# cloudflare/flow-pipeline

Hardware: AMD Instinct MI355X
Metric: FlowMessages/sec aggregated into flows_5m (higher is better)
Workload: dtype u64

## Files before the change

flow-pipeline_amd/csrc/flowagg.hip:

```cpp
#include <hip/hip_runtime.h>
#include <sched.h>
#include <hipcub/hipcub.hpp>

#include <algorithm>
#include <atomic>
#include <thread>
#include <chrono>
#include <cmath>
#include <condition_variable>
#include <functional>
#include <map>
#include <cstdio>
#include <cstdlib>
#include <cstring>
#include <ctime>
#include <memory>
#include <mutex>
#include <string>
#include <vector>

#include "../../include/flowagg.h"
#include "bucket_range.h"
#include "buffers.h"
#include "kernels.cuh"
// ... 66 lines not shown
        uint32_t* tail() const { return counts + wcounts_cap(counts); }
        uint32_t nwg = 0, wcapq = 0, wplog2 = 0, wmask = 0, wm = 0;
        size_t wregion = 0;
        uint64_t n = 0;
        uint32_t minb = 0, maxb = 0;
        bool minb_known = false;
    };
    std::vector<WChunk> wlog, wlog_free;
    bool wide_probed = false;
    bool wide_defer = false;
    uint64_t seen_wfold = 0;
    size_t wlog_max = 8;
    uint64_t wpot_total = 0, known_wpot = 0;
    uint64_t snap_wpot[NSNAP] = {};
    uint32_t wseg_budget = 0;
    uint32_t late_below = 0;
    uint64_t wlog_recorded = 0, wlog_folded = 0, wlog_replayed = 0, wlog_dropped = 0, wlog_wm_moves = 0, wlog_nomem_folds = 0;
    bool wide_scatter = true;
    uint64_t seen_wused = 0, seen_ok_w = 0;
    bool cms_atomic = false;
    bool cms_scatter_ok = false;
    int sink_mode = 0;
    int t8_mode = 0;
    uint64_t t8_wide_until = 0;
    uint64_t seen_misfit8 = 0, seen_ok = 0;
    uint64_t seen_retried = 0, seq_until = 0;
    int seq_mode = 0;
    uint64_t seen_agg_groups = 0, seen_agg_launches = 0;
    uint32_t agg_passes_forced = 0;
    uint32_t agg_passes = 1;
    unsigned stage_threads = 8;
    uint32_t par = 0;
    uint32_t seg_cap_limit = 0;
    uint32_t last_nwg = 0;
    uint32_t plog2 = PART_LOG2_MAX, wgpc_cap = 0;

    PinnedBuf<uint8_t> h_stage[2];
    hipEvent_t stage_ev[2] = {nullptr, nullptr};
    int stage_cur = 0;
    DevBuf<uint8_t> d_in[2];

    DevBuf<> col_block;
    ColumnPtrs cols{};

    DevBuf<> rc_buf;
    DevBuf<> rw_buf;
    DevBuf<> m_scratch;
    DevBuf<> m_out[2];
    DevBuf<> cut_buf;
    hipStream_t copy_stream = nullptr;
    hipStream_t cand_stream = nullptr;
    hipEvent_t cand_ev[2] = {nullptr, nullptr};
    DevBuf<> fs_scratch;
    DevBuf<> fs_off;
    DevBuf<> wl_scratch;
    DevBuf<> part_buf;
    DevBuf<unsigned int> part_cnt;
    DevBuf<> xch_buf;
    uint32_t group_members = 0;
    PinnedBuf<> h_rows;
    hipEvent_t copy_ev[2] = {nullptr, nullptr};

    DevBuf<unsigned long long> cms_src, cms_dst;
    size_t cms_words = 0;
    bool cms_dirty = false;
    DevBuf<unsigned long long> cms_src_m, cms_dst_m;
// ... 77 lines not shown
    a.tab = c->tab;
    a.mask = (1u << c->cap_log2) - 1;
    a.rlog2 = as_rlog2(c->cap_log2);
    a.spill = c->spill;
    a.spill_cap = c->spill_cap;
    a.ctr = c->d_ctr;
    a.exotic_idx = c->d_exotic;
    a.cms_src = c->cms_src;
    a.cms_dst = c->cms_dst;
    a.cms_depth = c->cfg.cms_depth;
    a.cms_wl2 = c->cfg.cms_width_log2;
    a.cms_seed = c->cfg.cms_seed;
    a.ks_src = c->ks_src;
    a.ks_dst = c->ks_dst;
    a.ks_mask = (1u << c->ks_log2) - 1;
    a.cand_src = c->cand_bits[0];
    a.cand_dst = c->cand_bits[1];
    a.cms_nrep = c->cand_state ? 1u : CMS_REPLICAS;
    a.cols = c->cols;
    a.dbg = c->dbg;
    a.tile_recs = BLOCK;
    a.retry_idx = c->d_exotic ? c->d_exotic + c->exotic_cap() : nullptr;
    a.key_sets = c->cfg.key_sets;
    a.wtab = c->wtab;
    a.wmask = (1u << c->wcap_log2) - 1;
    a.wplog2 = wide_plog2(c->wcap_log2);
    a.wspill = c->wspill;
    a.wspill_cap = c->wspill_cap;
    a.port_hist = c->port_hist;
    a.gran_recip = (1.0 / (double)c->gran) * (1.0 + 1.0 / 1099511627776.0);
    a.par = c->par;
    a.agg_passes = c->agg_passes_forced ? c->agg_passes_forced : c->agg_passes;
    a.late_below = c->late_below;
    return a;
}

template <class K>
static int grid_for(fa_ctx* c, K kernel, uint32_t n, uint32_t tile_recs) {
    uint32_t tiles = (n + tile_recs - 1) / tile_recs;
    int per_cu = 0;
    if (hipOccupancyMaxActiveBlocksPerMultiprocessor(&per_cu, kernel, BLOCK, 0) != hipSuccess || per_cu < 1)
        per_cu = 2;
    if (c->wgpc_cap && (int)c->wgpc_cap < per_cu) per_cu = (int)c->wgpc_cap;
    uint32_t g = std::min<uint32_t>((uint32_t)c->num_cus * (uint32_t)per_cu, SEG_MAX_NWG);
    return (int)std::max(1u, std::min(tiles, g));
}

extern "C" int fa_create(const fa_config* cfg_in, fa_ctx** out) {
    if (!cfg_in || !out) {
        g_create_error = "fa_create: null argument";
        return FA_ERR_ARG;
    }
    *out = nullptr;
    int ndev = 0;
    if (hipGetDeviceCount(&ndev) != hipSuccess || ndev <= 0) {
        g_create_error = "fa_create: no HIP device (libflowagg has no CPU fallback)";
        return FA_ERR_NO_DEVICE;
    }
    fa_config cfg = *cfg_in;
    if (cfg.window_secs == 0) cfg.window_secs = 300;
    if (cfg.table_capacity_log2 == 0) cfg.table_capacity_log2 = 20;
    if (cfg.cms_depth == 0) cfg.cms_depth = 4;
    if (cfg.cms_width_log2 == 0) cfg.cms_width_log2 = 20;
    if (cfg.key_sets == 0) cfg.key_sets = FA_KEYS_AS_PAIR;
    if (cfg.topk_capacity_log2 == 0) cfg.topk_capacity_log2 = 20;
    if (cfg.wide_capacity_log2 == 0) cfg.wide_capacity_log2 = 20;
    if (cfg.topk_track == 0) cfg.topk_track = 256;
    if (cfg.max_batch_records == 0) cfg.max_batch_records = AGG_MAX_BATCH;
    if (cfg.max_batch_records > AGG8_MAX_BATCH) cfg.max_batch_records = AGG8_MAX_BATCH;
    uint32_t gran = cfg.subwindow_secs ? cfg.subwindow_secs : cfg.window_secs;
    if (cfg.device < 0 || cfg.device >= ndev || gran < 60 || 86400 % gran != 0 ||
        cfg.window_secs % gran != 0 || 86400 % cfg.window_secs != 0 || cfg.table_capacity_log2 < 10 ||
        cfg.table_capacity_log2 > 30 || cfg.cms_depth > 16 || cfg.cms_width_log2 < 4 ||
        cfg.cms_width_log2 > 28 || (cfg.key_sets & ~63u) || cfg.topk_mode > FA_TOPK_CANDIDATES || cfg.topk_capacity_log2 < 8 || cfg.topk_capacity_log2 > 30 ||
        cfg.wide_capacity_log2 < 8 || cfg.wide_capacity_log2 > 30) {
        g_create_error = "fa_create: invalid configuration";
        return FA_ERR_ARG;
    }
    fa_ctx* c = new fa_ctx();
    c->cfg = cfg;
    c->gran = gran;
    c->cap_log2 = cfg.table_capacity_log2;
    if (const char* d = getenv("FA_DEBUG_FLAGS")) c->dbg = (uint32_t)strtoul(d, nullptr, 0);
    if (const char* d = getenv("FA_PLOG2")) c->plog2 = std::min<uint32_t>(PART_LOG2_MAX, std::max<uint32_t>(4, (uint32_t)atoi(d)));
    if (const char* d = getenv("FA_WGPC")) c->wgpc_cap = (uint32_t)atoi(d);
    if (const char* d = getenv("FA_SEG_CAP")) c->seg_cap_limit = std::max<uint32_t>(40u, (uint32_t)atoi(d) & ~7u);
    if (const char* d = getenv("FA_SINK")) c->sink_mode = !strcmp(d, "direct") ? 1 : !strcmp(d, "scatter") ? 2 : 0;
    if (const char* d = getenv("FA_CMS")) c->cms_atomic = !strcmp(d, "atomic");
    if (const char* d = getenv("FA_WIDE")) c->wide_mode = !strcmp(d, "atomic") ? 1 : !strcmp(d, "scatter") ? 2 : !strcmp(d, "log") ? 3 : 0;
    if (const char* d = getenv("FA_WIDE_LOG_CHUNKS")) c->wlog_max = (size_t)std::max(0, atoi(d));
    if (const char* d = getenv("FA_WSEG_BUDGET")) c->wseg_budget = (uint32_t)std::max(1, atoi(d));
    if (const char* d = getenv("FA_AGG_PASSES")) {
        const int v = atoi(d);
        c->agg_passes_forced = (v == 1 || v == 2 || v == 4 || v == 8) ? (uint32_t)v : 0u;
    }
    c->cms_scatter_ok = cms_scatterable(cfg.cms_depth, cfg.cms_width_log2);
    if (const char* d = getenv("FA_STAGE_THREADS")) c->stage_threads = (unsigned)std::min(64, std::max(1, atoi(d)));
    c->stage_threads = std::min(c->stage_threads, std::max(1u, std::thread::hardware_concurrency()));
    if (const char* d = getenv("FA_TUPLE")) c->t8_mode = !strcmp(d, "8") ? 1 : !strcmp(d, "16") ? 2 : 0;
    if (const char* d = getenv("FA_SEQ")) c->seq_mode = !strcmp(d, "1") ? 1 : !strcmp(d, "0") ? 2 : 0;
    auto bail = [&](const char* what, hipError_t e) {
        g_create_error = std::string("fa_create: ") + what + ": " + hipGetErrorString(e);
        fa_destroy(c);
        return e == hipErrorOutOfMemory ? FA_ERR_NOMEM : FA_ERR_HIP;
    };
    hipError_t e;
    if ((e = hipSetDevice(cfg.device)) != hipSuccess) return bail("hipSetDevice", e);
    {
        int v = 0;
        if (hipDeviceGetAttribute(&v, hipDeviceAttributeMultiprocessorCount, cfg.device) == hipSuccess && v > 0)
            c->num_cus = v;
    }
    if ((e = hipStreamCreateWithFlags(&c->stream, hipStreamNonBlocking)) != hipSuccess)
        return bail("hipStreamCreate", e);
    for (int i = 0; i < 2; i++)
        if ((e = hipEventCreateWithFlags(&c->stage_ev[i], hipEventDisableTiming)) != hipSuccess ||
            (e = hipEventCreateWithFlags(&c->copy_ev[i], hipEventDisableTiming)) != hipSuccess)
            return bail("hipEventCreate", e);
    for (int i = 0; i < fa_ctx::NSNAP; i++)
        if ((e = hipEventCreateWithFlags(&c->snap_ev[i], hipEventDisableTiming)) != hipSuccess) return bail("hipEventCreate", e);
    if (!c->h_snap.grow(sizeof(Counters) * fa_ctx::NSNAP)) return bail("hipHostMalloc", hipGetLastError());
    c->spill_cap = 2u * cfg.max_batch_records + (1u << 21);
    c->wide_per_record = ((cfg.key_sets & FA_KEYS_ADDR_PORT_PROTO) ? 1u : 0u) + ((cfg.key_sets & FA_KEYS_PORT_HIST) ? 2u : 0u) +
                         ((cfg.key_sets & FA_KEYS_MINUTE_SERIES) ? 1u : 0u);
    c->wspill_cap = (uint32_t)std::min<uint64_t>((uint64_t)c->wide_per_record * 2u * cfg.max_batch_records + (1u << 21), 1u << 25);
    size_t tab_bytes = sizeof(Slot) << c->cap_log2;
    if (!c->tab.grow(tab_bytes)) return bail("hipMalloc(table)", hipGetLastError());
    if ((e = hipMemsetAsync(c->tab, 0, tab_bytes, c->stream)) != hipSuccess) return bail("memset", e);
    if (!c->spill.grow(sizeof(SpillEntry) * c->spill_cap))
        return bail("hipMalloc(spill)", hipGetLastError());
    if (!c->d_ctr.grow(sizeof(Counters))) return bail("hipMalloc(ctr)", hipGetLastError());
    if ((e = hipMemsetAsync(c->d_ctr, 0, sizeof(Counters), c->stream)) != hipSuccess)
        return bail("memset", e);
    if (!c->h_ctr.grow(sizeof(Counters))) return bail("hipHostMalloc", hipGetLastError());
    if (cfg.key_sets & (FA_KEYS_SRCADDR_CMS | FA_KEYS_DSTADDR_CMS)) {
        c->cms_words = (size_t)cfg.cms_depth << cfg.cms_width_log2;
        if (cfg.key_sets & FA_KEYS_SRCADDR_CMS) {
            if (!c->cms_src.grow(c->cms_words * 8 * CMS_REPLICAS)) return bail("hipMalloc(cms)", hipGetLastError());
            if ((e = hipMemsetAsync(c->cms_src, 0, c->cms_words * 8 * CMS_REPLICAS, c->stream)) != hipSuccess)
                return bail("memset", e);
        }
        if (cfg.key_sets & FA_KEYS_DSTADDR_CMS) {
            if (!c->cms_dst.grow(c->cms_words * 8 * CMS_REPLICAS)) return bail("hipMalloc(cms)", hipGetLastError());
            if ((e = hipMemsetAsync(c->cms_dst, 0, c->cms_words * 8 * CMS_REPLICAS, c->stream)) != hipSuccess)
                return bail("memset", e);
        }
        if (cfg.topk_mode == FA_TOPK_CANDIDATES) {
            if ((e = hipStreamCreateWithFlags(&c->cand_stream, hipStreamNonBlocking)) != hipSuccess) return bail("hipStreamCreate(side stream)", e);
            for (int i = 0; i < 2; i++)
                if ((e = hipEventCreateWithFlags(&c->cand_ev[i], hipEventDisableTiming)) != hipSuccess) return bail("hipEventCreate", e);
        }
        c->ks_log2 = cfg.topk_capacity_log2;
        const size_t ks_bytes = sizeof(KeySlot) << c->ks_log2;
        if (cfg.key_sets & FA_KEYS_SRCADDR_CMS) {
            if (!c->ks_src.grow(ks_bytes)) return bail("hipMalloc(key set)", hipGetLastError());
            if ((e = hipMemsetAsync(c->ks_src, 0, ks_bytes, c->stream)) != hipSuccess) return bail("memset", e);
        }
        if (cfg.key_sets & FA_KEYS_DSTADDR_CMS) {
            if (!c->ks_dst.grow(ks_bytes)) return bail("hipMalloc(key set)", hipGetLastError());
            if ((e = hipMemsetAsync(c->ks_dst, 0, ks_bytes, c->stream)) != hipSuccess) return bail("memset", e);
        }
        if (cfg.topk_mode == FA_TOPK_CANDIDATES) {
            c->cand_bits_bytes = std::max<size_t>(c->cms_words / 8, 8) + 8;
            for (int d = 0; d < 2; d++)
                if (cfg.key_sets & (d ? FA_KEYS_DSTADDR_CMS : FA_KEYS_SRCADDR_CMS)) {
                    if (!c->cand_bits[d].grow(c->cand_bits_bytes)) return bail("hipMalloc(candidate bits)", hipGetLastError());
                    if ((e = hipMemsetAsync(c->cand_bits[d], 0, c->cand_bits_bytes, c->stream)) != hipSuccess) return bail("memset", e);
// ... 251 lines not shown
```

flow-pipeline_amd/csrc/ingest.cuh:

```cuda
#pragma once
#include <hip/hip_runtime.h>
#include <stdint.h>

#include "sinks.cuh"

#ifndef FA_FOLD_EVERY
#define FA_FOLD_EVERY 4
#endif
#ifndef FA_LT_KEEP
#define FA_LT_KEEP 8u
#endif
namespace fa {

struct NoHook {
    __device__ __forceinline__ void operator()() const {}
};
struct LaneTally {
    uint32_t ok = 0, direct = 0, second = 0, misfit8 = 0, late = 0;
    uint32_t tick = 0;
};
template <int MODE, uint32_t KEYSETS, uint32_t COLS, bool T8 = false, int CANDM = -1, class Hook = NoHook>
__device__ __forceinline__ void lane_work(const KArgs& a, LdsTable<LDS_SLOTS>& lt, LdsMinutes& lm, uint32_t* part_cnt, const uint32_t* tile,
                                          bool mine, uint32_t pos, uint32_t end, uint32_t rec_idx, uint32_t tb_base,
                                          LaneTally& tally, uint32_t& pmode, uint32_t& lt_seen, uint32_t& lt_hits,
                                          uint4* bins, uint32_t* bin_cnt, uint32_t& fill_out, Hook&& after_parse = Hook(),
                                          CmsLds* cl = nullptr, uint32_t* cms_scratch = nullptr, HotAddrs* hot = nullptr,
                                          uint32_t* wpart_cnt = nullptr, uint32_t* seq = nullptr) {
    constexpr uint32_t TB = bin_cap<T8, bin_line(KEYSETS)>();
    bool sure = false, framed_ok = false;
    Rec r;
    rec_clear(r);
    if (mine) {
        LdsSrc src{tile};
        framed_ok = true;
        if (a.framed && !(FA_DBG(a, DBG_NO_FRAME))) {
            uint32_t pl = 0;
// ... 471 lines not shown
};
template <>
struct HotAddrsOpt<false> {
    __device__ __forceinline__ HotAddrs* get() { return nullptr; }
};

template <uint32_t KEYSETS, bool T8, bool SEQ = false, int CANDM = -1>
__global__ __launch_bounds__(wtile_block<KEYSETS>(), wt_lean(KEYSETS) ? 6 : 4) void wtile_kernel(KArgs a) {
    constexpr uint32_t BL = bin_line(KEYSETS);
    constexpr uint32_t TB = bin_cap<T8, BL>();
    constexpr uint32_t COLS = cols_for_keysets<KEYSETS>();
    constexpr int WBLOCK = wtile_block<KEYSETS>();
    constexpr bool HAS_CMS = (KEYSETS & (FA_KEYS_SRCADDR_CMS | FA_KEYS_DSTADDR_CMS)) != 0;
    constexpr int WAVES = WBLOCK / 64;
    constexpr int WT_STRIDE = wtile_stride<KEYSETS>();
    __shared__ CmsLdsOpt<HAS_CMS> cms_lds;
    __shared__ HotAddrsOpt<HAS_CMS> hot_lds;
    __shared__ uint32_t cms_scratch_all[HAS_CMS ? WAVES * 16 : 1];
    __shared__ __attribute__((aligned(16))) uint32_t tiles[WAVES * WT_STRIDE / 4];
    __shared__ __attribute__((aligned(16))) uint4 bins[NPART_MAX * BL];
    __shared__ uint32_t bin_cnt[NPART_MAX];
    __shared__ uint32_t part_cnt[NPART_MAX];
    __shared__ uint32_t flush_scratch[WAVES * 16];
    constexpr bool HAS_APP = (KEYSETS & FA_KEYS_ADDR_PORT_PROTO) != 0;
    __shared__ uint32_t wpart_cnt[HAS_APP ? (1u << WIDE_PLOG2_MAX) + 2u : 1u];
    __shared__ LdsTable<LDS_SLOTS> lt;
    __shared__ LdsMinutes lm;
    constexpr bool HAS_SEQ = SEQ && KEYSETS == FA_KEYS_AS_PAIR;
    static_assert(!SEQ || KEYSETS == FA_KEYS_AS_PAIR, "the learnt-order variant exists for the flows_5m rollup alone");
    __shared__ uint32_t seq_all[HAS_SEQ ? WAVES * (SEQ_MAX + 2) : 1];

    const uint32_t tid = threadIdx.x, lane = tid & 63;
    const uint32_t wave = __builtin_amdgcn_readfirstlane(tid >> 6);
    if (HAS_SEQ && lane < 2) seq_all[wave * (SEQ_MAX + 2) + lane] = 0;
    if (KEYSETS & FA_KEYS_AS_PAIR) {
        lds_table_clear(lt);
        for (int i = tid; i < NPART_MAX; i += WBLOCK) {
            part_cnt[i] = 0;
            bin_cnt[i] = 0;
        }
    }
    if (KEYSETS & FA_KEYS_MINUTE_SERIES) lds_minutes_clear(lm);
    if (HAS_APP)
        for (int i = tid; i < (1 << WIDE_PLOG2_MAX) + 2; i += WBLOCK) wpart_cnt[i] = i < (1 << WIDE_PLOG2_MAX) ? 0u : 0xffffffffu;
    CmsLds* const cl = (HAS_CMS && (CANDM >= 0 || a.cseg)) ? cms_lds.get() : nullptr;
    HotAddrs* const hot = (HAS_CMS && (KEYSETS != KS_ALL || (a.key_sets & (FA_KEYS_SRCADDR_CMS | FA_KEYS_DSTADDR_CMS)))) ? hot_lds.get() : nullptr;
    if (HAS_CMS && cl)
        for (int i = tid; i < (int)(CMS_SETS * CMS_NPART); i += WBLOCK) {
            cl->bin_cnt[i] = 0;
            cl->part_cnt[i] = 0;
        }
    if (HAS_CMS && hot)
        for (int i = tid; i < (int)(CMS_SETS * HOT_SLOTS); i += WBLOCK) {
            const int set = i / HOT_SLOTS, sl = i % HOT_SLOTS;
            const size_t at = (size_t)blockIdx.x * (CMS_SETS * HOT_SLOTS) + i;
            const uint32_t tg = a.hot_seed_tag ? a.hot_seed_tag[at] : 0u;
            if (tg >= 2u) {
                const HotSeed sd = a.hot_seed[at];
                hot->lo[set][sl] = sd.lo;
                hot->hi[set][sl] = sd.hi;
                hot->w[set][sl] = 0;
            }
            hot->touched[set][sl] = 0;
            *hot->tag(set, sl) = tg >= 2u ? tg : 0u;
        }
    uint32_t* tile = tiles + wave * (WT_STRIDE / 4);

    LaneTally tally;
    uint32_t lt_seen = 0, lt_hits = 0, pmode = 0;
    uint32_t tb_base = 0;
    const uint32_t ntiles = (a.n + a.tile_recs - 1) / a.tile_recs;
    __shared__ uint32_t next_k;
    if (tid == 0) next_k = 2u * WAVES;
    const uint32_t wg_pos = (gridDim.x & 7u) == 0u ? (blockIdx.x & 7u) * (gridDim.x >> 3) + (blockIdx.x >> 3) : blockIdx.x;
    auto tile_after_next = [&]() {
        uint32_t k = 0;
        if (lane == 0) k = lds_add_rtn_u32(&next_k, 1u);
        return (uint32_t)__builtin_amdgcn_readfirstlane((int)k) * gridDim.x + wg_pos;
    };
    struct __attribute__((packed, aligned(4))) OffPair {
        uint32_t lo, hi;
    };
    struct Tile {
        uint32_t r0, nrec;
        uint32_t q0, q1;
    };
    auto tile_load = [&](uint32_t t) {
        Tile d{0, 0, 0, 0};
        if (t < ntiles) {
            d.r0 = t * a.tile_recs;
            d.nrec = min(a.tile_recs, a.n - d.r0);
            if (lane < d.nrec) {
                const OffPair v = *reinterpret_cast<const OffPair*>(a.off + d.r0 + lane);
                d.q0 = v.lo;
                d.q1 = v.hi;
            }
        }
        return d;
    };
    constexpr uint32_t CAP = (uint32_t)WT_STRIDE - 16u;
    auto issue_dma = [&](uint32_t lo, uint32_t hi) {
        const uint32_t cbase = lo & ~15u;
        const uint32_t nbytes = hi > cbase ? min(hi - cbase, CAP) : 0u;
        for (uint32_t o = lane * 16u; o < nbytes; o += 1024u)
            __builtin_amdgcn_global_load_lds((const __attribute__((address_space(1))) void*)(a.buf + cbase + o),
                                             (__attribute__((address_space(3))) void*)(tile + (o - lane * 16u) / 4u), 16, 0, 2);
    };
    Tile cur = tile_load(wave * gridDim.x + wg_pos);
    uint32_t cur_lo = (uint32_t)__builtin_amdgcn_readfirstlane((int)cur.q0);
    uint32_t cur_hi = cur.nrec ? min((uint32_t)__builtin_amdgcn_readlane((int)cur.q1, (int)(cur.nrec - 1u)), a.len) : 0u;
    bool live = lane < cur.nrec;
    __syncthreads();
    issue_dma(cur_lo, cur_hi);
    Tile nxt = tile_load((wave + WAVES) * gridDim.x + wg_pos);
    tb_base = probe_tb_base(a);
    if (blockIdx.x == 0 && tid == 0) a.ctr->tb_base = tb_base;
    uint32_t t2 = 0;
    bool t2_have = false;
    while (cur.nrec != 0) {
        dma_wait_all();
        if (!t2_have) {
            t2 = tile_after_next();
            t2_have = true;
        }
        const uint32_t cbase = cur_lo & ~15u;
        const bool valid = live && cur.q1 >= cur.q0 && cur.q0 >= cur_lo && cur.q1 <= cur_hi;
        const bool staged = valid && cur.q1 - cbase <= CAP;
        bool rest = valid && !staged;
        const bool hopeless = (live && !valid) || (rest && cur.q0 == cur_lo);
        if (FA_ANY(hopeless)) {
            if (hopeless) {
                unsigned int j = atomicAdd(&a.ctr->exotic_count[a.par], 1u);
                a.exotic_idx[j] = cur.r0 + lane;
            }
            rest = rest && !hopeless;
        }
        uint32_t fill = 0xffffffffu;
        lane_work<MODE_INGEST, KEYSETS, COLS, T8, CANDM>(a, lt, lm, part_cnt, tile, staged, cur.q0 - cbase, cur.q1 - cbase, cur.r0 + lane, tb_base, tally,
                                                  pmode, lt_seen, lt_hits, bins, bin_cnt, fill, NoHook(), cl, cms_scratch_all + (HAS_CMS ? wave * 16 : 0), hot,
                                                  (HAS_APP && a.wseg) ? wpart_cnt : nullptr, HAS_SEQ ? seq_all + wave * (SEQ_MAX + 2) : nullptr);
        if ((KEYSETS & FA_KEYS_AS_PAIR) && a.seg) bins_flush<T8, BL>(a, bins, bin_cnt, part_cnt, flush_scratch + wave * 16, fill, tb_base, tally.direct);
        const unsigned long long restm = __builtin_amdgcn_ballot_w64(rest);
        if (restm != 0ull) {
            live = rest;
            cur_lo = (uint32_t)__builtin_amdgcn_readlane((int)cur.q0, (int)__builtin_ctzll(restm));
            issue_dma(cur_lo, cur_hi);
            continue;
        }
        t2_have = false;
        cur = nxt;
        cur_lo = (uint32_t)__builtin_amdgcn_readfirstlane((int)cur.q0);
        cur_hi = cur.nrec ? min((uint32_t)__builtin_amdgcn_readlane((int)cur.q1, (int)(cur.nrec - 1u)), a.len) : 0u;
        live = lane < cur.nrec;
        issue_dma(cur_lo, cur_hi);
        nxt = tile_load(t2);
// ... 97 lines not shown
        __syncthreads();
        for (int i = tid; i < (1 << a.wplog2); i += WBLOCK) a.wseg_counts[(size_t)i * a.nwg + blockIdx.x] = min(wpart_cnt[i], a.wcapq);
        if (tid == 0 && wpart_cnt[1u << WIDE_PLOG2_MAX] != 0xffffffffu) {
            atomicMin(&a.ctr->wtb_min, wpart_cnt[1u << WIDE_PLOG2_MAX]);
            atomicMin(&a.ctr->wtb_nmax, wpart_cnt[(1u << WIDE_PLOG2_MAX) + 1u]);
        }
    }
    if (KEYSETS & FA_KEYS_AS_PAIR) {
        __syncthreads();
        for (int i0 = 0; i0 < LDS_SLOTS; i0 += WBLOCK) {
            const int i = i0 + tid;
            Slot* sp = nullptr;
            unsigned long long b = 0, p = 0, c = 0;
            if (i < LDS_SLOTS) {
                const unsigned long long k0 = lt.k0[i], k1 = lt.k1[i];
                b = lt.bytes[i];
                p = lt.packets[i];
                c = lt.count[i];
                if (k0 != 0 && k1 != 0 && c != 0) {
                    sp = table_find_or_claim(a, k0, k1, key_hash(k0, k1));
                    if (!sp) spill_park(a, k0, k1, b, p, c);
                }
            }
            quad_atomic_update(sp, b, p, c);
        }
        if (a.seg)
            for (int i = tid; i < (1 << a.plog2); i += WBLOCK) {
                const uint32_t w = part_cnt[i];
                a.seg_counts[(size_t)i * a.nwg + blockIdx.x] = min((w & 0xffffu) * TB, a.capf);
                a.seg_counts[((size_t)NPART_MAX + i) * a.nwg + blockIdx.x] = min(w >> 16, a.capb);
            }
    }
    block_counters_add(bin_cnt, a.ctr, tally);
}

template <int MODE, uint32_t KEYSETS>
__device__ __forceinline__ void exotic_pass(const KArgs& a) {
    const uint32_t cnt = a.ctr->exotic_count[a.par];
    for (uint32_t j = blockIdx.x * BLOCK + threadIdx.x; j < cnt; j += gridDim.x * BLOCK) {
        uint32_t idx = a.exotic_idx[j];
        const uint32_t x0 = a.off[idx], x1 = a.off[idx + 1];
        const uint8_t* p = a.buf + min(x0, a.len);
        const uint8_t* end = a.buf + min(x1, a.len);
        bool ok = x1 >= x0 && x1 <= a.len;
        if (ok && a.framed) ok = frame_generic(p, end);
        Rec r;
        if (ok)
            ok = parse_generic(p, end, r);
        if (!ok) rec_clear(r);
        atomicAdd(&a.ctr->slow, 1ull);
        if (MODE == MODE_DECODE) {
            store_columns(a.cols, idx, r, ok ? 0 : 1);
            continue;
        }
        if (!ok) {
            atomicAdd(&a.ctr->bad, 1ull);
            continue;
        }
        atomicAdd(&a.ctr->ok, 1ull);
        const uint32_t tb = (uint32_t)r.time_received / a.gran;
        if (tb < a.late_below) atomicAdd(&a.ctr->late, 1ull);
        if (ks_on<KEYSETS>(a, FA_KEYS_AS_PAIR)) {
            uint64_t k0, k1;
            pack_key(tb, r.src_as, r.dst_as, r.etype, k0, k1);
            agg_global(a, k0, k1, key_hash(k0, k1), r.bytes, r.packets, 1);
        }
// ... 49 lines not shown
            }
        }
        if (MODE == MODE_DECODE) {
            if (sure) store_columns(a.cols, idx, r, 0);
            continue;
        }
        n_ok += sure ? 1 : 0;
        const uint32_t tb = time_bucket(a, (uint32_t)r.time_received);
        if (sure && tb < a.late_below) atomicAdd(&a.ctr->late, 1ull);
        if (ks_on<KEYSETS>(a, FA_KEYS_AS_PAIR)) {
            uint64_t k0, k1;
            pack_key(tb, r.src_as, r.dst_as, r.etype, k0, k1);
            uint64_t b = r.bytes, p = r.packets, c = 1;
            bool valid = sure;
            wave_combine<16, 2>(valid, k0, k1, b, p, c);
            if (valid) agg_global(a, k0, k1, key_hash(k0, k1), b, p, c);
        }
        if (sure && (KEYSETS & (FA_KEYS_SRCADDR_CMS | FA_KEYS_DSTADDR_CMS))) {
            const uint64_t w = r.bytes * r.sampling_rate;
            if (ks_on<KEYSETS>(a, FA_KEYS_SRCADDR_CMS)) {
                cms_add(a.cms_src, a.cms_depth, a.cms_wl2, a.cms_seed, r.src, w, a.cms_nrep);
                keyset_offer(a, 0u, r.src);
            }
            if (ks_on<KEYSETS>(a, FA_KEYS_DSTADDR_CMS)) {
                cms_add(a.cms_dst, a.cms_depth, a.cms_wl2, a.cms_seed, r.dst, w, a.cms_nrep);
                keyset_offer(a, 1u, r.dst);
            }
        }
        if (sure && (KEYSETS & FA_KEYS_WIDE)) wide_sink_slow<KEYSETS>(a, r, tb);
    }
    if (blockIdx.x == 0 && threadIdx.x == 0) {
        a.ctr->exotic_count[a.par ^ 1u] = 0;
        a.ctr->retry_count[a.par ^ 1u] = 0;
    }
    if (MODE == MODE_INGEST) {
        uint64_t tot = wave_sum_u64(n_ok);
        if (__lane_id() == 0 && tot) {
            atomicAdd(&a.ctr->ok, (unsigned long long)tot);
            atomicAdd(&a.ctr->retried, (unsigned long long)tot);
        }
    }
}

}
```

flow-pipeline_amd/csrc/ingest_host.inc:

```

template <uint32_t KS, bool SEQ = false, int CANDM = -1>
static void launch_wtile(fa_ctx* c, const KArgs& a, const LaunchPlan& p) {
    const dim3 g(p.grid), b(wtile_block<KS>());
    if (p.t8) hipLaunchKernelGGL((wtile_kernel<KS, true, SEQ, CANDM>), g, b, 0, c->stream, a);
    else hipLaunchKernelGGL((wtile_kernel<KS, false, SEQ, CANDM>), g, b, 0, c->stream, a);
}
template <uint32_t KS>
static void launch_wave_tiles(fa_ctx* c, const KArgs& a, const LaunchPlan& p) {
    if constexpr ((KS & (FA_KEYS_SRCADDR_CMS | FA_KEYS_DSTADDR_CMS)) != 0u && KS != KS_ALL)
        if (p.cms_segments) return c->cand_state ? launch_wtile<KS, false, 1>(c, a, p) : launch_wtile<KS, false, 0>(c, a, p);
    if constexpr (KS == 1u)
        if (p.seq_variant) return launch_wtile<1u, true>(c, a, p);
    launch_wtile<KS>(c, a, p);
}
static int cand_boundary(fa_ctx* c) {
    HIPCHK(c, hipMemsetAsync(c->cand_state, 0, 2 * sizeof(CandState), c->stream));
    const dim3 gs(CAND_SCAN_BLOCKS, 2), gb(256, 2);
    hipLaunchKernelGGL(cand_scan_kernel, gs, dim3(256), 0, c->stream, c->ks_src, c->ks_dst, 1u << c->ks_log2, (const unsigned long long*)c->cms_src,
                       (const unsigned long long*)c->cms_dst, c->cfg.cms_depth, c->cfg.cms_width_log2, c->cfg.cms_seed, c->cand_state, c->cand_chunkmax);
    hipLaunchKernelGGL(cand_bits_kernel, gb, dim3(256), 0, c->stream, (const KeySlot*)c->ks_src, (const KeySlot*)c->ks_dst, (const unsigned long long*)c->cms_src,
                       (const unsigned long long*)c->cms_dst, c->cfg.cms_depth, c->cfg.cms_width_log2, c->cfg.topk_track, std::max(c->ks_log2, 8u) - 2u, c->cand_state,
                       c->cand_bits[0], c->cand_bits[1]);
    return FA_OK;
}
template <int MODE>
static int launch_tiles(fa_ctx* c, KArgs& a, const LaunchPlan& p, fa_ctx::LaunchEvents* ev) {
    if (p.wave_tiles && (MODE != MODE_INGEST || !(p.variant & FA_KEYS_AS_PAIR) || !a.seg)) return fail(c, FA_ERR_ARG, "internal: wave tiles without tuple segments");
    const dim3 b(BLOCK), ge(std::min(256u, (a.n + BLOCK - 1) / BLOCK));
    a.par = c->par;
    c->par ^= 1u;
    if (ev) (void)hipEventRecord(ev->e0, c->stream);
    if (p.seq_variant) c->stats.learnt_order_launches += 1;
    if (p.wave_tiles) c->stats.wave_tile_launches += 1;
    if (p.t8) c->stats.compact_tuple_launches += 1;
    if (p.wide_segments) HIPCHK(c, hipMemsetAsync(&c->d_ctr->wtb_min, 0xff, 2 * sizeof(unsigned int), c->stream));
    auto launch = [&](auto variant) {
        constexpr uint32_t KS = decltype(variant)::value;
        if (!p.wave_tiles) {
// ... 618 lines not shown
```

flow-pipeline_amd/csrc/launch_plan.h:

```cpp
#pragma once
#include <algorithm>
#include <cmath>
#include <type_traits>
#include <utility>

#include "sinks.cuh"

namespace fa {

constexpr uint32_t ks_variant(uint32_t key_sets) { return (key_sets >= 1u && key_sets <= 7u) || key_sets == 9u ? key_sets : KS_ALL; }
template <class F>
decltype(auto) with_variant(uint32_t variant, F&& f) {
    switch (variant) {
    case 1u: return f(std::integral_constant<uint32_t, 1u>{});
    case 2u: return f(std::integral_constant<uint32_t, 2u>{});
    case 3u: return f(std::integral_constant<uint32_t, 3u>{});
    case 4u: return f(std::integral_constant<uint32_t, 4u>{});
    case 5u: return f(std::integral_constant<uint32_t, 5u>{});
    case 6u: return f(std::integral_constant<uint32_t, 6u>{});
    case 7u: return f(std::integral_constant<uint32_t, 7u>{});
    case 9u: return f(std::integral_constant<uint32_t, 9u>{});
    default: return f(std::integral_constant<uint32_t, KS_ALL>{});
    }
}

inline uint32_t tile_recs_for(size_t bytes, size_t n) {
    if (n == 0) return BLOCK;
    const double r = ((double)TILE_BYTES - 15.0) / ((double)bytes / (double)n + 0.5);
    return r >= (double)BLOCK ? (uint32_t)BLOCK : r < 1.0 ? 1u : (uint32_t)r;
}
inline uint32_t wtile_recs_for(size_t bytes, size_t n, uint32_t variant) {
    const double avg = (double)bytes / (double)n, cap = (double)wt_stride(variant) - 16.0 - 15.0;
    const double r = (cap - 2.0 * 12.0 * std::sqrt(std::min(cap / avg, (double)WT_RECS))) / avg;
    return r >= (double)WT_RECS ? (uint32_t)WT_RECS : r < 1.0 ? 1u : (uint32_t)r;
}
inline int wtile_grid(uint32_t n, uint32_t tile_recs, uint32_t variant, uint32_t num_cus) {
    const uint32_t waves = (uint32_t)(wt_lean(variant) ? WBLOCK : WBLOCK_CMS) / 64u;
    const uint32_t wgs = ((n + tile_recs - 1) / tile_recs + waves - 1) / waves;
    return (int)std::max(1u, std::min(wgs, num_cus * (wt_lean(variant) ? (uint32_t)WT_WG_PER_CU : 1u)));
}

struct LaunchPlan {
    uint32_t variant = 1u;
    uint32_t tile_recs = BLOCK;
    int grid = 1;
    bool wave_tiles = false;
    bool t8 = false;
    bool seq_variant = false;
    bool cms_segments = false;
    bool wide_segments = false;
    bool wlog = false;
    bool side = false;
};

}
```

flow-pipeline_amd/csrc/sinks.cuh:

```cuda
#pragma once
#include <hip/hip_runtime.h>
#include <stdint.h>

#include "gen.cuh"
#include "table.cuh"
#include "wide.cuh"
#include "wire.cuh"

namespace fa {

constexpr int BLOCK = 256;
constexpr int TILE_BYTES = 21760;
constexpr int TILE_PAD = 112;
constexpr int TILE_STRIDE = TILE_BYTES + TILE_PAD;
constexpr int LDS_SLOTS = 64;
constexpr int LDS_PROBES = 2;
constexpr int PART_LOG2_MAX = 8;
constexpr int NPART_MAX = 1 << PART_LOG2_MAX;
#ifndef FA_WBLOCK
#define FA_WBLOCK 768
#endif
#ifndef FA_WT_STRIDE
#define FA_WT_STRIDE 4864
#endif
// ... 27 lines not shown

enum { MODE_INGEST = 0, MODE_DECODE = 1 };
constexpr uint32_t KS_ALL = 0xFFu;
constexpr uint32_t FA_KEYS_WIDE = FA_KEYS_ADDR_PORT_PROTO | FA_KEYS_PORT_HIST | FA_KEYS_MINUTE_SERIES;
constexpr uint32_t PORT_DENSE = 65536;
#ifndef FA_ABLATE
#define FA_ABLATE 0
#endif
#ifndef FA_TL_WINDOW
#define FA_TL_WINDOW 256u
#endif
#define FA_DBG(a, flags) (FA_ABLATE != 0 && ((a).dbg & (flags)) != 0)
enum { DBG_NO_SINK = 1, DBG_LOOP_PARSER = 2, DBG_NO_LDS_TABLE = 4, DBG_NO_GLOBAL = 8, DBG_NO_PARSE = 16, DBG_NO_TUPLE_STORE = 32,
       DBG_AGG_NO_LDS = 64, DBG_AGG_NO_FLUSH = 128, DBG_AGG_NO_SLOW = 256, DBG_DMA_NO_NT = 512, DBG_TIMING = 1024, DBG_TUPLE_NT = 2048, DBG_TUPLE_SC = 4096, DBG_NO_LANE_OFF = 8192, DBG_SYNTH_TILES = 16384, DBG_NOT_MINE = 32768, DBG_NO_SECOND = 65536, DBG_NO_FRAME = 131072, DBG_NO_KEYSET = 262144, DBG_NO_CMS = 524288, DBG_NO_HOT = 1048576, DBG_CMS_TUPLE_LOCAL = 268435456 , DBG_NO_SINGLES = 134217728 , DBG_TUPLE_LOCAL = 67108864 , DBG_CAND_NO_SET = 33554432 , DBG_AGG_ATOMIC_FLUSH = 2097152 ,
       DBG_AGG8_TIMING = 8388608 ,
       DBG_CMS_TIMING = 4194304  };

struct SpillEntry {
    unsigned long long k0, k1, bytes, packets, count;
};

struct Counters {
    unsigned long long ok, bad, slow, spill_lost, used, direct, retried;
    unsigned long long misfit8;
    unsigned int exotic_count[2], retry_count[2];
    unsigned int spill_count, rows_count, ks_overflow, ks_rows;
    unsigned int tb_base, wtb_min, wtb_nmax, pad;
    unsigned long long t_wait, t_work, t_tiles, t_total;
    unsigned long long wfold_n;
    unsigned long long wused, wspill_lost;
    unsigned int wspill_count, wrows_count;
    unsigned long long agg_groups, agg_launches;
    unsigned long long late;
};

struct __attribute__((aligned(32))) KeySlot {
    unsigned long long tag, lo, hi, pad;
};
constexpr unsigned long long KS_CLAIMED = 1ull << 63, KS_READY = 1ull << 62;
struct TopkRow {
    unsigned long long lo, hi, weight;
};
constexpr uint32_t TK_BINS = 2048;
__host__ __device__ __forceinline__ uint32_t topk_bin(unsigned long long est) {
    if (est < 64ull) return (uint32_t)est;
#if defined(__HIP_DEVICE_COMPILE__)
    const uint32_t e = 63u - (uint32_t)__clzll((long long)est);
#else
    const uint32_t e = 63u - (uint32_t)__builtin_clzll(est);
#endif
    return ((e - 4u) << 5) | ((uint32_t)(est >> (e - 5u)) & 31u);
}
__host__ __device__ __forceinline__ unsigned long long topk_bin_floor(uint32_t b) {
    if (b < 64u) return b;
    const uint32_t e = (b >> 5) + 4u;
    return (1ull << e) | ((unsigned long long)(b & 31u) << (e - 5u));
}

struct CandState {
    unsigned int hist[TK_BINS];
    unsigned int sel[4];
    unsigned long long total;
    unsigned long long theta;
};

struct ColumnPtrs {
    uint64_t *time_received, *time_flow_start, *sampling_rate, *bytes, *packets;
    uint32_t *sequence_num, *src_as, *dst_as, *etype, *proto, *src_port, *dst_port;
    uint4 *sampler_address, *src_addr, *dst_addr;
    uint8_t* status;
};

struct HotSeed;
struct KArgs {
    const uint8_t* buf;
    const uint32_t* off;
    uint32_t n;
    uint32_t len;
    uint32_t framed;
    uint32_t gran;
    Slot* tab;
    uint32_t mask;
    SpillEntry* spill;
    uint32_t spill_cap;
    Counters* ctr;
    uint32_t* exotic_idx;
    unsigned long long* cms_src;
    unsigned long long* cms_dst;
    uint32_t cms_depth, cms_wl2;
    uint64_t cms_seed;
    KeySlot* ks_src;
    KeySlot* ks_dst;
    const uint32_t* cand_src;
    const uint32_t* cand_dst;
    uint32_t cms_nrep;
    uint32_t ks_mask;
    ColumnPtrs cols;
    uint32_t tile_recs;
    uint32_t dbg;
    uint32_t* retry_idx;
    double gran_recip;
    uint4* seg;
    uint32_t* seg_counts;
    uint32_t capq;
    uint32_t capf, capb;
    uint32_t nwg;
    unsigned long long region;
    uint32_t plog2;
    uint32_t par;
    uint32_t rlog2;
    uint32_t agg_passes;
    uint4* cseg;
    uint32_t* cseg_counts;
    uint32_t ccapq, ccapf, ccapb;
    unsigned long long cregion;
    uint32_t cms_sub;
    HotSeed* hot_seed;
    uint32_t* hot_seed_tag;
    uint32_t hot_epoch;
    uint32_t* cms_psize;
    uint32_t key_sets;
    WSlot* wtab;
    uint32_t wmask;
    WSpillEntry* wspill;
    uint32_t wspill_cap;
    uint4* wseg;
    uint32_t* wseg_counts;
    uint32_t wcapq;
    uint32_t wplog2;
    unsigned long long wregion;
    ulonglong2* port_hist;
    uint32_t late_below;
};

__device__ __forceinline__ KArgs cold_args() {
#if defined(__HIP_DEVICE_COMPILE__)
    const KArgs* p = (const KArgs*)__builtin_amdgcn_kernarg_segment_ptr();
    asm volatile("" : "+s"(p));
    return *p;
#else
    return KArgs{};
#endif
}

__device__ __forceinline__ WArgs wargs(const KArgs& a) {
    return WArgs{a.wtab, a.wmask, a.wmask >> a.wplog2, a.wspill, a.wspill_cap, &a.ctr->wspill_count, &a.ctr->wspill_lost, &a.ctr->wused};
}
template <uint32_t KEYSETS>
__device__ __forceinline__ bool ks_on(const KArgs& a, uint32_t x) {
    return (KEYSETS & x) != 0 && (KEYSETS != KS_ALL || (a.key_sets & x) != 0);
}

__device__ __forceinline__ void agg_global(const KArgs& a, uint64_t k0, uint64_t k1, uint32_t h,
                                           uint64_t b, uint64_t p, uint64_t c) {
    uint32_t i = as_home(k0, k1, h, a.mask, a.rlog2);
    for (int probe = 0; probe < FA_MAX_PROBES; probe++, i = as_next(i, a.mask, a.rlog2)) {
        Slot* s = &a.tab[i];
        unsigned long long c0 = s->k0;
        if (c0 == 0) c0 = atomicCAS(&s->k0, 0ull, (unsigned long long)k0);
        if (c0 != 0 && c0 != k0) continue;
        unsigned long long c1 = s->k1;
        if (c1 == 0) {
            c1 = atomicCAS(&s->k1, 0ull, (unsigned long long)k1);
            if (c1 == 0) count_created(&a.ctr->used);
        }
// ... 659 lines not shown
```

Baseline: 50.27 billion.

## Add global tile pool with shrinking run lengths to balance workgroup tails

The wave-tile ingest kernel now splits tiles into a static round-robin prefix and a shared tail pool. Workgroups claim the pool through a global atomic counter in runs that shrink across three levels, so late tiles go to whichever workgroups finish first. This targets tail imbalance where some workgroups finish much later than others. It adds global atomics, an LDS ring with spin-waits, and scheduling logic in the hot loop. Per-workgroup timing instrumentation is included behind a debug flag.

Result: no change. 50.40 billion, median of 6 (+0.2%).

```diff
diff --git a/flow-pipeline_amd/csrc/flowagg.hip b/flow-pipeline_amd/csrc/flowagg.hip
--- a/flow-pipeline_amd/csrc/flowagg.hip
+++ b/flow-pipeline_amd/csrc/flowagg.hip
@@ -122,6 +122,8 @@
     unsigned stage_threads = 8;
     uint32_t par = 0;
     uint32_t seg_cap_limit = 0;
+    uint32_t pool_share = TILE_POOL_SHARE;
+    DevBuf<unsigned long long> wg_times;
     uint32_t last_nwg = 0;
     uint32_t plog2 = PART_LOG2_MAX, wgpc_cap = 0;
 
@@ -265,6 +267,8 @@
     a.par = c->par;
     a.agg_passes = c->agg_passes_forced ? c->agg_passes_forced : c->agg_passes;
     a.late_below = c->late_below;
+    a.pool_share = c->pool_share;
+    a.wg_times = c->wg_times;
     return a;
 }
 
@@ -318,6 +322,7 @@
     if (const char* d = getenv("FA_PLOG2")) c->plog2 = std::min<uint32_t>(PART_LOG2_MAX, std::max<uint32_t>(4, (uint32_t)atoi(d)));
     if (const char* d = getenv("FA_WGPC")) c->wgpc_cap = (uint32_t)atoi(d);
     if (const char* d = getenv("FA_SEG_CAP")) c->seg_cap_limit = std::max<uint32_t>(40u, (uint32_t)atoi(d) & ~7u);
+    if (const char* d = getenv("FA_TILE_POOL")) c->pool_share = (uint32_t)std::min(16, std::max(0, atoi(d)));
     if (const char* d = getenv("FA_SINK")) c->sink_mode = !strcmp(d, "direct") ? 1 : !strcmp(d, "scatter") ? 2 : 0;
     if (const char* d = getenv("FA_CMS")) c->cms_atomic = !strcmp(d, "atomic");
     if (const char* d = getenv("FA_WIDE")) c->wide_mode = !strcmp(d, "atomic") ? 1 : !strcmp(d, "scatter") ? 2 : !strcmp(d, "log") ? 3 : 0;
@@ -366,6 +371,7 @@
     if ((e = hipMemsetAsync(c->d_ctr, 0, sizeof(Counters), c->stream)) != hipSuccess)
         return bail("memset", e);
     if (!c->h_ctr.grow(sizeof(Counters))) return bail("hipHostMalloc", hipGetLastError());
+    if (FA_ABLATE != 0 && (c->dbg & DBG_TIMING) && !c->wg_times.grow(sizeof(unsigned long long) * (1 + WG_TIMES_MAX))) return bail("hipMalloc(workgroup times)", hipGetLastError());
     if (cfg.key_sets & (FA_KEYS_SRCADDR_CMS | FA_KEYS_DSTADDR_CMS)) {
         c->cms_words = (size_t)cfg.cms_depth << cfg.cms_width_log2;
         if (cfg.key_sets & FA_KEYS_SRCADDR_CMS) {
diff --git a/flow-pipeline_amd/csrc/ingest.cuh b/flow-pipeline_amd/csrc/ingest.cuh
--- a/flow-pipeline_amd/csrc/ingest.cuh
+++ b/flow-pipeline_amd/csrc/ingest.cuh
@@ -2,6 +2,7 @@
 #include <hip/hip_runtime.h>
 #include <stdint.h>
 
+#include "launch_plan.h"
 #include "sinks.cuh"
 
 #ifndef FA_FOLD_EVERY
@@ -539,6 +540,7 @@
 
     const uint32_t tid = threadIdx.x, lane = tid & 63;
     const uint32_t wave = __builtin_amdgcn_readfirstlane(tid >> 6);
+    if (FA_DBG(a, DBG_TIMING) && a.wg_times && tid == 0) atomicMin(&a.wg_times[0], (unsigned long long)wall_clock64());
     if (HAS_SEQ && lane < 2) seq_all[wave * (SEQ_MAX + 2) + lane] = 0;
     if (KEYSETS & FA_KEYS_AS_PAIR) {
         lds_table_clear(lt);
@@ -578,12 +580,53 @@
     uint32_t tb_base = 0;
     const uint32_t ntiles = (a.n + a.tile_recs - 1) / a.tile_recs;
     __shared__ uint32_t next_k;
-    if (tid == 0) next_k = 2u * WAVES;
+    __shared__ unsigned long long pool_ring[8];
+    __shared__ TileSchedule sched;
+    constexpr uint32_t POOL_BIT = 0x80000000u;
+    const uint32_t k_static = TileSchedule::static_rounds(ntiles, gridDim.x, a.pool_share);
+    if (tid == 0) {
+        next_k = 2u * WAVES + (POOL_BIT - k_static);
+        sched = TileSchedule::make(ntiles, gridDim.x, WAVES, a.pool_share);
+    }
+    if (tid < 8) pool_ring[tid] = 0;
     const uint32_t wg_pos = (gridDim.x & 7u) == 0u ? (blockIdx.x & 7u) * (gridDim.x >> 3) + (blockIdx.x >> 3) : blockIdx.x;
-    auto tile_after_next = [&]() {
+    const uint32_t wg_off = wg_pos - (POOL_BIT - k_static) * gridDim.x;
+    auto draw_k = [&]() {
         uint32_t k = 0;
         if (lane == 0) k = lds_add_rtn_u32(&next_k, 1u);
-        return (uint32_t)__builtin_amdgcn_readfirstlane((int)k) * gridDim.x + wg_pos;
+        return (uint32_t)__builtin_amdgcn_readfirstlane((int)k);
+    };
+    auto pool_tile = [&](uint32_t j) {
+        volatile unsigned long long* const ring = pool_ring;
+        for (;;) {
+            const uint32_t q = j / (uint32_t)WAVES, pos = j - q * (uint32_t)WAVES;
+            if (j == 0u && lane == 0) {
+                uint32_t r0 = 0xfffffffeu;
+                if (sched.nruns != 0u) {
+                    const KArgs ca = cold_args();
+                    r0 = atomicAdd(&ca.ctr->tile_head[ca.par], 2u);
+                }
+                ring[0] = (1ull << 32) | r0;
+                ring[1] = (2ull << 32) | (r0 + 1u);
+            }
+            unsigned long long e;
+            while ((uint32_t)__builtin_amdgcn_readfirstlane((int)(uint32_t)((e = ring[q & 7u]) >> 32)) != q + 1u) __builtin_amdgcn_s_sleep(1);
+            const uint32_t r = (uint32_t)__builtin_amdgcn_readfirstlane((int)(uint32_t)e);
+            if (pos == 0u && q != 0u && lane == 0) {
+                uint32_t r1 = 0xffffffffu;
+                if (r < sched.nruns) {
+                    const KArgs ca = cold_args();
+                    r1 = atomicAdd(&ca.ctr->tile_head[ca.par], 1u);
+                }
+                ring[(q + 1u) & 7u] = ((unsigned long long)(q + 2u) << 32) | r1;
+            }
+            uint32_t lo = 0, hi = 0;
+            const bool have = sched.run(r, lo, hi);
+            const uint32_t len = (uint32_t)__builtin_amdgcn_readfirstlane((int)(have ? hi - lo : 0xffffffffu));
+            if (len == 0xffffffffu) return ntiles;
+            if (pos < len) return (uint32_t)__builtin_amdgcn_readfirstlane((int)lo) + pos;
+            j = draw_k() & ~POOL_BIT;
+        }
     };
     struct __attribute__((packed, aligned(4))) OffPair {
         uint32_t lo, hi;
@@ -598,7 +641,7 @@
             d.r0 = t * a.tile_recs;
             d.nrec = min(a.tile_recs, a.n - d.r0);
             if (lane < d.nrec) {
-                const OffPair v = *reinterpret_cast<const OffPair*>(a.off + d.r0 + lane);
+                const OffPair v = *reinterpret_cast<const OffPair*>(cold_args().off + d.r0 + lane);
                 d.q0 = v.lo;
                 d.q1 = v.hi;
             }
@@ -613,13 +656,19 @@
             __builtin_amdgcn_global_load_lds((const __attribute__((address_space(1))) void*)(a.buf + cbase + o),
                                              (__attribute__((address_space(3))) void*)(tile + (o - lane * 16u) / 4u), 16, 0, 2);
     };
-    Tile cur = tile_load(wave * gridDim.x + wg_pos);
+    const bool pool_first = k_static < 2u * WAVES;
+    Tile cur = tile_load(pool_first ? ntiles : wave * gridDim.x + wg_pos);
+    __syncthreads();
+    uint32_t t_second = (wave + WAVES) * gridDim.x + wg_pos;
+    if (pool_first) {
+        cur = tile_load(wave < k_static ? wave * gridDim.x + wg_pos : pool_tile(wave - k_static));
+        if (wave + WAVES >= k_static) t_second = pool_tile(wave + WAVES - k_static);
+    }
     uint32_t cur_lo = (uint32_t)__builtin_amdgcn_readfirstlane((int)cur.q0);
     uint32_t cur_hi = cur.nrec ? min((uint32_t)__builtin_amdgcn_readlane((int)cur.q1, (int)(cur.nrec - 1u)), a.len) : 0u;
     bool live = lane < cur.nrec;
-    __syncthreads();
     issue_dma(cur_lo, cur_hi);
-    Tile nxt = tile_load((wave + WAVES) * gridDim.x + wg_pos);
+    Tile nxt = tile_load(t_second);
     tb_base = probe_tb_base(a);
     if (blockIdx.x == 0 && tid == 0) a.ctr->tb_base = tb_base;
     uint32_t t2 = 0;
@@ -627,7 +676,9 @@
     while (cur.nrec != 0) {
         dma_wait_all();
         if (!t2_have) {
-            t2 = tile_after_next();
+            const uint32_t k = draw_k();
+            t2 = k * gridDim.x + wg_off;
+            if (k & POOL_BIT) t2 = pool_tile(k & ~POOL_BIT);
             t2_have = true;
         }
         const uint32_t cbase = cur_lo & ~15u;
@@ -791,6 +842,10 @@
             }
     }
     block_counters_add(bin_cnt, a.ctr, tally);
+    if (FA_DBG(a, DBG_TIMING) && a.wg_times) {
+        __syncthreads();
+        if (tid == 0 && blockIdx.x < WG_TIMES_MAX) a.wg_times[1u + blockIdx.x] = (unsigned long long)wall_clock64();
+    }
 }
 
 template <int MODE, uint32_t KEYSETS>
@@ -906,6 +961,7 @@
     if (blockIdx.x == 0 && threadIdx.x == 0) {
         a.ctr->exotic_count[a.par ^ 1u] = 0;
         a.ctr->retry_count[a.par ^ 1u] = 0;
+        a.ctr->tile_head[a.par ^ 1u] = 0;
     }
     if (MODE == MODE_INGEST) {
         uint64_t tot = wave_sum_u64(n_ok);
diff --git a/flow-pipeline_amd/csrc/ingest_host.inc b/flow-pipeline_amd/csrc/ingest_host.inc
--- a/flow-pipeline_amd/csrc/ingest_host.inc
+++ b/flow-pipeline_amd/csrc/ingest_host.inc
@@ -1,9 +1,47 @@
 
+static void tile_tail_record(fa_ctx* c, const KArgs& a, const LaunchPlan& p) {
+    const uint32_t g = std::min<uint32_t>((uint32_t)p.grid, WG_TIMES_MAX);
+    std::vector<unsigned long long> t(1 + (size_t)g);
+    if (hipStreamSynchronize(c->stream) != hipSuccess || hipMemcpy(t.data(), c->wg_times, t.size() * sizeof(t[0]), hipMemcpyDeviceToHost) != hipSuccess) return;
+    struct Stat { double mean, p50, p99, max; };
+    auto stat = [](std::vector<double>& v) {
+        std::sort(v.begin(), v.end());
+        double s = 0;
+        for (double x : v) s += x;
+        const size_t n = v.size();
+        return n ? Stat{s / (double)n, v[n / 2], v[std::min(n - 1, (size_t)((double)n * 0.99))], v[n - 1]} : Stat{0, 0, 0, 0};
+    };
+    std::vector<double> all, by[8];
+    for (uint32_t b = 0; b < g; b++) {
+        const double us = (double)(t[1 + b] - t[0]) * 0.01;
+        all.push_back(us);
+        by[b & 7u].push_back(us);
+    }
+    const Stat s = stat(all);
+    std::string out = "{\"kernel\": \"wtile_kernel\", \"variant\": " + std::to_string(p.variant) + ", \"n\": " + std::to_string(a.n) + ", \"grid\": " + std::to_string(g) +
+                      ", \"tile_recs\": " + std::to_string(a.tile_recs) + ", \"pool_share\": " + std::to_string(a.pool_share);
+    char buf[256];
+    snprintf(buf, sizeof buf, ", \"duration_us\": %.2f, \"end_us\": {\"mean\": %.2f, \"p50\": %.2f, \"p99\": %.2f, \"max\": %.2f}, \"tail_frac\": %.4f, \"by_xcd\": [", s.max, s.mean, s.p50,
+             s.p99, s.max, s.max > 0 ? (s.max - s.mean) / s.max : 0.0);
+    out += buf;
+    for (int x = 0; x < 8; x++) {
+        const Stat sx = stat(by[x]);
+        snprintf(buf, sizeof buf, "%s{\"mean\": %.2f, \"p50\": %.2f, \"p99\": %.2f, \"max\": %.2f}", x ? ", " : "", sx.mean, sx.p50, sx.p99, sx.max);
+        out += buf;
+    }
+    out += "]}\n";
+    const char* path = getenv("FA_TILE_TAIL_OUT");
+    FILE* f = path ? fopen(path, "a") : nullptr;
+    fputs(out.c_str(), f ? f : stderr);
+    if (f) fclose(f);
+}
 template <uint32_t KS, bool SEQ = false, int CANDM = -1>
 static void launch_wtile(fa_ctx* c, const KArgs& a, const LaunchPlan& p) {
     const dim3 g(p.grid), b(wtile_block<KS>());
+    const bool tail = FA_ABLATE != 0 && (c->dbg & DBG_TIMING) && c->wg_times && hipMemsetAsync(c->wg_times, 0xff, sizeof(unsigned long long), c->stream) == hipSuccess;
     if (p.t8) hipLaunchKernelGGL((wtile_kernel<KS, true, SEQ, CANDM>), g, b, 0, c->stream, a);
     else hipLaunchKernelGGL((wtile_kernel<KS, false, SEQ, CANDM>), g, b, 0, c->stream, a);
+    if (tail) tile_tail_record(c, a, p);
 }
 template <uint32_t KS>
 static void launch_wave_tiles(fa_ctx* c, const KArgs& a, const LaunchPlan& p) {
diff --git a/flow-pipeline_amd/csrc/launch_plan.h b/flow-pipeline_amd/csrc/launch_plan.h
--- a/flow-pipeline_amd/csrc/launch_plan.h
+++ b/flow-pipeline_amd/csrc/launch_plan.h
@@ -40,6 +40,53 @@
     return (int)std::max(1u, std::min(wgs, num_cus * (wt_lean(variant) ? (uint32_t)WT_WG_PER_CU : 1u)));
 }
 
+constexpr uint32_t TILE_POOL_SHARE = 2u;
+constexpr int TILE_POOL_LEVELS = 3;
+struct TileSchedule {
+    uint32_t ntiles, grid, rounds, pool0, nruns;
+    uint32_t sec_tile[TILE_POOL_LEVELS + 1];
+    uint32_t sec_run[TILE_POOL_LEVELS + 1];
+    uint32_t sec_len[TILE_POOL_LEVELS];
+
+    __host__ __device__ static uint32_t static_rounds(uint32_t ntiles, uint32_t grid, uint32_t share) {
+        const uint32_t pool = (uint32_t)(((unsigned long long)ntiles * (share < 16u ? share : 16u)) >> 4);
+        return (ntiles - pool + grid - 1u) / grid;
+    }
+    __host__ __device__ static TileSchedule make(uint32_t ntiles, uint32_t grid, uint32_t waves, uint32_t share) {
+        TileSchedule s;
+        s.ntiles = ntiles;
+        s.grid = grid;
+        s.rounds = static_rounds(ntiles, grid, share);
+        const unsigned long long first = (unsigned long long)s.rounds * grid;
+        s.pool0 = first < ntiles ? (uint32_t)first : ntiles;
+        uint32_t at = s.pool0, run = 0;
+        for (int i = 0; i < TILE_POOL_LEVELS; i++) {
+            const uint32_t len = (waves >> i) ? (waves >> i) : 1u;
+            const unsigned long long keep = (unsigned long long)grid * len;
+            uint32_t end = ntiles;
+            if (i + 1 < TILE_POOL_LEVELS) end = (ntiles > keep && ntiles - (uint32_t)keep > at) ? ntiles - (uint32_t)keep : at;
+            s.sec_tile[i] = at;
+            s.sec_run[i] = run;
+            s.sec_len[i] = len;
+            run += (end - at + len - 1u) / len;
+            at = end;
+        }
+        s.sec_tile[TILE_POOL_LEVELS] = at;
+        s.sec_run[TILE_POOL_LEVELS] = run;
+        s.nruns = run;
+        return s;
+    }
+    __host__ __device__ uint32_t static_tile(uint32_t k, uint32_t p) const { return k * grid + p; }
+    __host__ __device__ bool run(uint32_t r, uint32_t& lo, uint32_t& hi) const {
+        if (r >= nruns) return false;
+        int i = 0;
+        while (i + 1 < TILE_POOL_LEVELS && r >= sec_run[i + 1]) i++;
+        lo = sec_tile[i] + (r - sec_run[i]) * sec_len[i];
+        hi = lo + sec_len[i] < sec_tile[i + 1] ? lo + sec_len[i] : sec_tile[i + 1];
+        return true;
+    }
+};
+
 struct LaunchPlan {
     uint32_t variant = 1u;
     uint32_t tile_recs = BLOCK;
diff --git a/flow-pipeline_amd/csrc/sinks.cuh b/flow-pipeline_amd/csrc/sinks.cuh
--- a/flow-pipeline_amd/csrc/sinks.cuh
+++ b/flow-pipeline_amd/csrc/sinks.cuh
@@ -83,6 +83,7 @@
     unsigned int wspill_count, wrows_count;
     unsigned long long agg_groups, agg_launches;
     unsigned long long late;
+    unsigned int tile_head[2];
 };
 
 struct __attribute__((aligned(32))) KeySlot {
@@ -123,6 +124,7 @@
 };
 
 struct HotSeed;
+constexpr uint32_t WG_TIMES_MAX = 4096;
 struct KArgs {
     const uint8_t* buf;
     const uint32_t* off;
@@ -182,6 +184,8 @@
     unsigned long long wregion;
     ulonglong2* port_hist;
     uint32_t late_below;
+    uint32_t pool_share;
+    unsigned long long* wg_times;
 };
 
 __device__ __forceinline__ KArgs cold_args() {
```
